# iqbal-lab-org/gramtools

Hardware: AMD Instinct MI355X
Metric: 150bp reads quasimapped/sec (whole node); bit-exact coverage (higher is better)
Workload: dtype u32

## Files before the change

gramtools_amd/csrc/gmx_engine_cover_kernels.h:

```cpp
#pragma once
struct CoverAcc {
  uint32_t *acc;
  uint32_t *log;
  uint32_t *log_cursor;
  uint32_t log_cap;
  uint32_t *scratch_big;
  uint32_t n_lanes_big;
  int rng_mode;
  uint32_t log_sites;
  uint32_t *heap;
  uint64_t heap_words;
  const uint32_t *status;
  uint32_t n_tasks;
  unsigned long long *stats;
};

#define GMX_LOG_PAD 0xFFFFFFFFu
#ifdef GMX_LOOP_STATS
__device__ unsigned long long gmx_cover_stats[6 * 16];
__device__ unsigned long long gmx_coop_stats[6 * 8];
extern "C" int gmx_debug_coop_stats(unsigned long long *out, int reset) {
  if (hipMemcpyFromSymbol(out, HIP_SYMBOL(gmx_coop_stats), sizeof(gmx_coop_stats)) != hipSuccess) return -1;
  if (reset) {
    unsigned long long z[6 * 8] = {0};
// ... 798 lines not shown
    gmx_cover_single_rec<NESTED>(ix, o, acc, recs_in[i], o.cover_overflow_list, 4u);
}

__global__ void gmx_stats_limbs_kernel(unsigned long long *stats, uint32_t *limbs, int recombine) {
  const uint32_t t = threadIdx.x;
  if (!recombine) {
    if (t < 20) limbs[t] = (uint32_t)((stats[t >> 2] >> (16 * (t & 3))) & 0xFFFFull);
    else if (t < 32) limbs[t] = 0;
  } else if (t < 5) {
    unsigned long long v = 0;
    for (int l = 3; l >= 0; --l) v = (v << 16) + limbs[4 * t + l];
    stats[t] = v;
  }
}

#define GMX_PACK_READS 128
#define GMX_PACK_IN_BYTES (24 * 1024)
#define GMX_PACK_OUT_PAIRS (GMX_PACK_IN_BYTES / 32 + GMX_PACK_READS + 8)
typedef uint32_t __attribute__((aligned(1))) gmx_u32_unaligned;
__device__ __forceinline__ void pack4(uint32_t x, uint32_t &lo, uint32_t &hi, uint32_t &bad) {
  uint32_t y = x - 0x01010101u;
  bad |= ((y & ~x & 0x80808080u) | (y & 0xFCFCFCFCu));
  lo = (((y & 0x01010101u) * 0x01020408u) >> 24) & 0xFu;
  hi = ((((y >> 1) & 0x01010101u) * 0x01020408u) >> 24) & 0xFu;
}
__device__ __forceinline__ uint2 pack_tail(const uint8_t *p, uint32_t rem, uint32_t &bad) {
  uint2 out = make_uint2(0, 0);
  for (uint32_t j = 0; j < rem; ++j) {
    uint32_t x = p[j];
    if (x < 1 || x > 4) bad = 1;
// ... 94 lines not shown
```

gramtools_amd/csrc/gmx_engine_host.h:

```cpp
#pragma once
#define HIP_TRY(expr)                                                                      \
  do {                                                                                     \
    hipError_t _e = (expr);                                                                \
    if (_e != hipSuccess) {                                                                \
      gmx_set_error(std::string(#expr) + ": " + hipGetErrorString(_e));                    \
      return GMX_EHIP;                                                                     \
    }                                                                                      \
  } while (0)

enum : int { GMX_TK_SEED = 0, GMX_TK_FILTER0, GMX_TK_FILTER1, GMX_TK_SINGLE, GMX_TK_EXTEND2, GMX_TK_UNPACK, GMX_TK_N };
static_assert(GMX_TK_N <= GMX_TIMED_KERNELS, "gmx_timing::kernel_ms holds GMX_TIMED_KERNELS entries");

struct gmx_engine {
  gmx_engine_opts opts;
  GmxIndexView dview;
  std::vector<void *> allocs;
  uint64_t index_bytes = 0;
  uint32_t *d_fused = nullptr, *d_limbs = nullptr;
  size_t n_fused = 0, n_acc = 0;
  std::vector<uint32_t> phys_allele, phys_pb, phys_grouped;
  std::vector<uint32_t> hit_fix;
  unsigned long long *d_stats = nullptr;
  uint32_t *d_error = nullptr;
  uint32_t *d_log = nullptr, *d_log_cursor = nullptr;
  uint32_t log_cap = 0;
  uint32_t n_allele = 0, n_pb = 0, n_grouped = 0;
  uint64_t cap_reads = 0;
  uint8_t *d_skip = nullptr;
  uint2 *d_packed = nullptr;
  uint64_t cap_packed = 0;
  uint32_t *d_status = nullptr, *d_n_final = nullptr, *d_mapped = nullptr, *d_overflow = nullptr, *d_counters = nullptr;
  uint32_t *d_general_rest = nullptr;
  uint32_t *d_single_rest = nullptr;
  bool cover_jump = false;
  uint32_t *d_task_lists = nullptr;
  GmxSeed *d_alive_seed = nullptr;
  uint32_t *d_alive = nullptr, *d_dead = nullptr, *d_dead2 = nullptr;
  uint64_t *d_seed_cursor = nullptr;
// ... 129 lines not shown
    return GMX_OK;
  }
  int upload(const uint32_t **dst, const gmx::WordBuf &src) {
    uint32_t *q = nullptr;
    int rc = alloc(&q, src.size(), false);
    if (rc) return rc;
    const size_t piece = (size_t)1 << 28;
    for (size_t at = 0; at < src.size(); at += piece)
      HIP_TRY(hipMemcpy(q + at, src.data() + at, std::min(piece, src.size() - at) * sizeof(uint32_t), hipMemcpyHostToDevice));
    index_bytes += src.size() * sizeof(uint32_t);
    *dst = q;
    return GMX_OK;
  }
};

static hipError_t gmx_event_wait(hipEvent_t ev) {
  static const bool spin = getenv("GMX_WAIT_SPIN") != nullptr;
  if (spin) return hipEventSynchronize(ev);
  const auto t0 = std::chrono::steady_clock::now();
  for (bool napping = false;;) {
    const hipError_t q = hipEventQuery(ev);
    if (q != hipErrorNotReady) return q;
    (void)hipGetLastError();
    if (!napping) {
      napping = std::chrono::steady_clock::now() - t0 > std::chrono::microseconds(60);
      continue;
    }
    struct timespec ts = {0, 50 * 1000};
    nanosleep(&ts, nullptr);
  }
}

static int gmx_quiesce(gmx_engine *e) {
  if (!e->ev_wait) HIP_TRY(hipEventCreateWithFlags(&e->ev_wait, hipEventDisableTiming | hipEventBlockingSync));
  hipStream_t streams[5] = {e->last_stream, e->copy_stream, e->side_stream, e->side2_stream, e->copy_stream2};
  for (int i = 0; i < 5; ++i) {
    if (i > 0 && !streams[i]) continue;
    bool seen = false;
    for (int j = 0; j < i; ++j) seen = seen || streams[j] == streams[i];
    if (seen) continue;
// ... 9 lines not shown
  HIP_TRY(hipEventRecord(e->ev_zeroed, stream));
  ++e->zero_epoch;
  return GMX_OK;
}
static int twin_join(gmx_engine *e, hipStream_t stream) {
  gmx_engine *tw = e->twin;
  if (!tw || !e->twin_in_flight) return GMX_OK;
  if (!e->ev_twin_done) HIP_TRY(hipEventCreateWithFlags(&e->ev_twin_done, hipEventDisableTiming));
  HIP_TRY(hipEventRecord(e->ev_twin_done, tw->main_stream));
  HIP_TRY(hipStreamWaitEvent(stream, e->ev_twin_done, 0));
  return GMX_OK;
}
static int flush_reset(gmx_engine *e) {
  if (!e->reset_pending) return GMX_OK;
  e->reset_pending = false;
  HIP_TRY(hipMemsetAsync(e->d_fused, 0, (e->n_fused + 32) * 4, e->reset_stream));
  return note_zeroed(e, e->reset_stream);
}

static int log_settle(gmx_engine *e);
static int gmx_log_drain(gmx_engine *e, uint64_t keep_below) {
  int frc = flush_reset(e);
  if (frc) return frc;
  HIP_TRY(hipDeviceSynchronize());
  uint32_t used = 0;
  HIP_TRY(hipMemcpy(&used, e->d_log_cursor, 4, hipMemcpyDeviceToHost));
  used = std::min(used, e->log_cap);
  e->log_reads_since = 0;
  e->log_known = used;
  if (used <= keep_below) return GMX_OK;
  std::vector<uint32_t> w(used);
  HIP_TRY(hipMemcpy(w.data(), e->d_log, (size_t)used * 4, hipMemcpyDeviceToHost));
  std::vector<uint32_t> key;
  for (size_t i = 0; i < w.size();) {
    if (w[i] == GMX_LOG_PAD) {
      ++i;
      continue;
    }
    if (i + 2 > w.size() || i + 2 + (size_t)w[i + 1] > w.size()) {
      gmx_set_error("grouped-allele-count log: malformed record at word " + std::to_string(i) + " of " + std::to_string(w.size()));
      return GMX_EREF;
    }
    key.assign(1, w[i]);
    key.insert(key.end(), w.begin() + i + 2, w.begin() + i + 2 + w[i + 1]);
    e->log_counts[key] += 1;
    i += 2 + w[i + 1];
  }
  HIP_TRY(hipMemset(e->d_log_cursor, 0, 4));
  e->log_known = 0;
  return GMX_OK;
}

template <class Env, int LIST>
static void launch_cover_lds(gmx_engine *e, hipStream_t stream, const BatchView &b, const SearchOut &o, const CoverAcc &acc,
                             bool after_coop = false) {
  static const uint32_t lanes_env = getenv("GMX_COVER_LANES") ? (uint32_t)atoi(getenv("GMX_COVER_LANES")) : 0u;
  const uint32_t lanes = lanes_env ? std::min(lanes_env, gmx_cover_lds_lanes<Env>()) : gmx_cover_lds_lanes<Env>();
  const size_t lds = (size_t)GmxScratchFixed<Env>::total * lanes * sizeof(uint32_t);
  const uint32_t per_cu = std::min<uint32_t>((uint32_t)(160 * 1024 / lds), 32u);
  hipLaunchKernelGGL((gmx_cover_kernel<Env, LIST>), dim3(e->n_cus * per_cu), dim3(64), lds, stream, e->dview, b, o, e->big,
                     acc, lanes, after_coop ? 1u : 0u);
}

// ... 69 lines not shown
  if ((rc = e->alloc(&e->d_inst_width, e->big.max_slots, false))) return rc;
  if ((rc = e->alloc(&e->d_inst_serial, e->big.max_slots, false))) return rc;
  if ((rc = e->alloc(&e->d_general_serial, n_tasks, false))) return rc;
  if ((rc = e->alloc(&e->d_big_serial, e->big.max_slots, false))) return rc;
  if ((rc = e->alloc(&e->d_overflow3, 2 * n_tasks, false))) return rc;
  if ((rc = e->alloc(&e->d_inst_arena, (size_t)e->inst_cap * GMX_FAST_ARENA, false))) return rc;
  if ((rc = e->alloc(&e->d_inst_states, (size_t)e->inst_cap * GMX_INST_STATES, false))) return rc;
  e->cap_reads = cap;
  return GMX_OK;
}

struct GmxDeviceIndex {
  uint64_t serial = 0;
  int device = 0;
  GmxIndexView view{};
  std::vector<void *> allocs;
  uint64_t bytes = 0;
  int refs = 0;
};
static std::mutex g_dev_index_mu;
static std::vector<GmxDeviceIndex *> g_dev_indexes;
static void gmx_dev_index_release(GmxDeviceIndex *d) {
  if (!d) return;
  std::lock_guard<std::mutex> lk(g_dev_index_mu);
  if (--d->refs > 0) return;
  for (void *p : d->allocs) (void)hipFree(p);
  g_dev_indexes.erase(std::remove(g_dev_indexes.begin(), g_dev_indexes.end(), d), g_dev_indexes.end());
  delete d;
}

static int engine_create(const gmx_index *ixh, const gmx_engine_opts *opts_in, gmx_engine *primary, gmx_engine **out);
int gmx_engine_create(const gmx_index *ixh, const gmx_engine_opts *opts_in, gmx_engine **out) try {
  int rc = engine_create(ixh, opts_in, nullptr, out);
  if (rc) return rc;
  gmx_engine *e = *out;
  const gmx::HostIndex &h = gmx_index_host(ixh);
  const bool can = !e->log_sites && e->shared_index && !getenv("GMX_NO_INDEX_SHARE");
  bool want = can && (h.is_nested || e->index_bytes >= (2ull << 30));
  if (const char *tw = getenv("GMX_TWIN")) want = can && atoi(tw) != 0;
  if (want) {
    gmx_engine *t = nullptr;
    if (engine_create(ixh, &e->opts, e, &t) == GMX_OK) {
      e->twin = t;
// ... 96 lines not shown
  }
  e->dview = v;
  e->n_allele = h.n_allele_slots;
  e->n_pb = h.n_pb_slots;
  e->n_grouped = h.n_grouped_slots;
  {
    e->n_acc = ((size_t)h.n_acc_slots + 63) / 64 * 64;
    e->n_fused = e->n_acc + 32;
    if (primary)
      e->d_fused = primary->d_fused;
    else
      rc |= e->alloc(&e->d_fused, e->n_fused + 32, true);
    e->d_limbs = e->d_fused ? e->d_fused + e->n_acc : nullptr;
    e->d_stats = e->d_fused ? reinterpret_cast<unsigned long long *>(e->d_fused + e->n_fused) : nullptr;
    e->d_log_cursor = e->d_fused ? e->d_fused + e->n_fused + 16 : nullptr;
    rc |= e->alloc(&e->d_error, 2, true);
    e->phys_allele = h.phys_allele;
    e->phys_pb = h.phys_pb;
    e->phys_grouped = h.phys_grouped;
    e->hit_fix = h.hit_fix;
  }
  for (const GmxSite &st : h.sites) e->log_sites = e->log_sites || st.grouped_off == GMX_GROUPED_LOG;
  {
    uint64_t n_jump = 0;
    for (const GmxSiteGeo &g : h.site_geo) n_jump += (g.flags & GMX_SITE_JUMP) ? 1u : 0u;
    e->cover_jump = !h.is_nested && 2 * n_jump > h.site_geo.size() && !getenv("GMX_NO_COVER_JUMP");
    if (getenv("GMX_NO_COVER_JUMP")) e->dview.site_geo = nullptr;
  }
  {
    uint64_t cap = opts.log_cap_words ? opts.log_cap_words
                   : e->log_sites     ? (1ull << 26)
                                      : 64;
    e->log_cap = (uint32_t)std::min<uint64_t>(cap, 0xFFFFFF00ull);
  }
  if (primary)
// ... 84 lines not shown
  }
  if (!primary && e->seed_cursor && !rc && !getenv("GMX_NO_SA_CTX")) {
    uint32_t *sc = nullptr;
    if (e->alloc(&sc, h.sa.size(), false) == GMX_OK) {
      hipLaunchKernelGGL(gmx_sa_ctx_kernel, dim3(8192), dim3(256), 0, nullptr, e->dview.sa, e->dview.text, (uint64_t)h.sa.size(), sc);
      if (hipDeviceSynchronize() == hipSuccess) {
        e->dview.sa_ctx = sc;
        e->index_bytes += h.sa.size() * sizeof(uint32_t);
      }
    } else {
      (void)hipGetLastError();
    }
  }
  if (!primary && e->seed_cursor && !rc && !getenv("GMX_NO_SEED_SIDE") && h.seed_words.size() > 1) {
    uint32_t *side = nullptr;
    const size_t n_side = h.seed_words.size() / 4 + 2;
    if (e->alloc(&side, n_side, false) == GMX_OK) {
      hipLaunchKernelGGL(gmx_seed_side_kernel, dim3(8192), dim3(256), 0, nullptr, e->dview.seeds, (uint64_t)h.seeds.size(), e->dview.seed_words,
                         e->dview.seed_shift, side);
      if (h.kmer_size2)
        hipLaunchKernelGGL(gmx_seed_side_kernel, dim3(8192), dim3(256), 0, nullptr, e->dview.seeds2, (uint64_t)h.seeds2.size(), e->dview.seed_words,
                           e->dview.seed_shift, side);
      if (hipDeviceSynchronize() == hipSuccess) {
        e->dview.seed_side = side;
        e->index_bytes += n_side * sizeof(uint32_t);
      }
    } else {
      (void)hipGetLastError();
    }
  }
  auto make_stream = [&](hipStream_t *st) -> bool {
// ... 31 lines not shown
  (void)hipSetDevice(e->opts.device);
  (void)hipDeviceSynchronize();
  if (e->twin) gmx_engine_destroy(e->twin);
  e->twin = nullptr;
  if (e->main_stream) (void)hipStreamDestroy(e->main_stream);
  if (e->ev_zeroed) (void)hipEventDestroy(e->ev_zeroed);
  if (e->ev_twin_done) (void)hipEventDestroy(e->ev_twin_done);
  if (e->side_stream) (void)hipStreamDestroy(e->side_stream);
  if (e->side2_stream) (void)hipStreamDestroy(e->side2_stream);
  if (e->ev_fork2) (void)hipEventDestroy(e->ev_fork2);
  if (e->ev_side1) (void)hipEventDestroy(e->ev_side1);
  if (e->ev_filter) (void)hipEventDestroy(e->ev_filter);
  if (e->ev_fork) (void)hipEventDestroy(e->ev_fork);
  if (e->ev_join) (void)hipEventDestroy(e->ev_join);
  if (e->ev_wait) (void)hipEventDestroy(e->ev_wait);
  if (e->copy_stream) (void)hipStreamDestroy(e->copy_stream);
  if (e->copy_stream2) (void)hipStreamDestroy(e->copy_stream2);
  if (e->h_log_state) (void)hipHostFree(e->h_log_state);
  if (e->ev_log_state) (void)hipEventDestroy(e->ev_log_state);
  for (auto &sl : e->pslot) {
    if (sl.copied) (void)hipEventDestroy(sl.copied);
    if (sl.done) (void)hipEventDestroy(sl.done);
  }
  for (auto &sl : e->stage) {
    if (sl.copied) (void)hipEventDestroy(sl.copied);
    if (sl.done) (void)hipEventDestroy(sl.done);
    if (sl.h_offsets) (void)hipHostFree(sl.h_offsets);
    if (sl.h_seeds) (void)hipHostFree(sl.h_seeds);
  }
  for (void *p : e->allocs) (void)hipFree(p);
  gmx_dev_index_release(e->shared_index);
  delete e;
} GMX_GUARD_VOID("gmx_engine_destroy")

int gmx_engine_reset(gmx_engine *e) try {
  HIP_TRY(hipSetDevice(e->opts.device));
  e->reset_pending = false;
  HIP_TRY(hipDeviceSynchronize());
  HIP_TRY(hipMemset(e->d_fused, 0, (e->n_fused + 32) * 4));
  HIP_TRY(hipMemset(e->d_error, 0, 8));
  HIP_TRY(hipMemset(e->d_counters, 0, GMX_N_COUNTERS * GMX_CNT_STRIDE * 4));
  if (e->twin) {
    HIP_TRY(hipMemset(e->twin->d_error, 0, 8));
    HIP_TRY(hipMemset(e->twin->d_counters, 0, GMX_N_COUNTERS * GMX_CNT_STRIDE * 4));
    e->twin_in_flight = false;
  }
  e->log_counts.clear();
  e->log_known = e->log_reads_since = 0;
  e->log_state_pending = false;
  return GMX_OK;
} GMX_GUARD_INT("gmx_engine_reset")

int gmx_engine_reset_async(gmx_engine *e, void *hip_stream) try {
  HIP_TRY(hipSetDevice(e->opts.device));
  hipStream_t st = (hipStream_t)hip_stream;
  int frc = flush_reset(e);
  if (frc) return frc;
  if ((frc = twin_join(e, st))) return frc;
  e->twin_in_flight = false;
  e->reset_pending = true;
  e->reset_stream = st;
  e->log_counts.clear();
  e->log_known = e->log_reads_since = 0;
  e->log_state_pending = false;
  return GMX_OK;
} GMX_GUARD_INT("gmx_engine_reset_async")

static bool gmx_ab_no_filter() {
  static const bool off = getenv("GMX_AB_NO_FILTER") != nullptr;
  return off;
}
static void launch_filter(gmx_engine *e, hipStream_t st, dim3 task_grid, const BatchView &b, const SearchOut &o, int pass,
                          hipEvent_t t0 = nullptr, hipEvent_t t1 = nullptr) {
  if (gmx_ab_no_filter()) return;
  if (e->filter_lds_words)
    hipExtLaunchKernelGGL(gmx_filter_lds_kernel, dim3(e->n_cus), dim3(GMX_FILTER_LDS_THREADS), e->filter_lds_words * 4,
// ... 8 lines not shown
  if (!e->h_log_state) {
    HIP_TRY(hipHostMalloc(reinterpret_cast<void **>(&e->h_log_state), 4 * sizeof(uint32_t), hipHostMallocDefault));
    HIP_TRY(hipEventCreateWithFlags(&e->ev_log_state, hipEventDisableTiming));
  }
  HIP_TRY(hipMemcpyAsync(e->h_log_state + 0, e->d_log_cursor, 4, hipMemcpyDeviceToHost, stream));
  HIP_TRY(hipMemcpyAsync(e->h_log_state + 1, e->d_counters + GMX_CNT_LOG_RETRY * GMX_CNT_STRIDE, 4, hipMemcpyDeviceToHost, stream));
  HIP_TRY(hipMemcpyAsync(e->h_log_state + 2, e->d_counters + GMX_CNT_LOG_RETRY_RECS * GMX_CNT_STRIDE, 4, hipMemcpyDeviceToHost, stream));
  HIP_TRY(hipMemcpyAsync(e->h_log_state + 3, e->d_counters + GMX_CNT_LOG_RETRY_HUGE * GMX_CNT_STRIDE, 4, hipMemcpyDeviceToHost, stream));
  HIP_TRY(hipEventRecord(e->ev_log_state, stream));
  e->log_state_pending = true;
  return GMX_OK;
}

static int launch_log_replay(gmx_engine *e, hipStream_t stream) {
  const int in = e->log_retry_side, out = in ^ 1;
  SearchOut o = e->last_o;
  o.log_retry_list = e->d_log_retry[out];
  o.log_retry_recs = e->d_log_retry_recs[out];
  o.log_retry_huge = e->d_log_retry_huge[out];
  o.cover_overflow_list = e->d_log_retry[in];
  hipLaunchKernelGGL(gmx_log_replay_setup_kernel, dim3(1), dim3(1024), 0, stream, o, e->d_log_retry_huge[in]);
  if (e->dview.is_nested)
    hipLaunchKernelGGL(gmx_cover_single_replay_kernel<true>, dim3(e->n_cus * 4), dim3(GMX_BLOCK), 0, stream, e->dview, e->last_b, o, e->last_acc,
                     e->d_log_retry_recs[in]);
  else
    hipLaunchKernelGGL(gmx_cover_single_replay_kernel<false>, dim3(e->n_cus * 4), dim3(GMX_BLOCK), 0, stream, e->dview, e->last_b, o, e->last_acc,
                     e->d_log_retry_recs[in]);
  hipLaunchKernelGGL((gmx_cover_kernel<CoverEnvBig, 1>), dim3(e->cover_big_lanes / 64), dim3(64), e->last_big_lds, stream, e->dview,
                     e->last_b, o, e->big, e->last_acc, 64u, 0u);
  HIP_TRY(hipGetLastError());
// ... 9 lines not shown
  uint64_t before = ~0ull;
  for (int round = 0;; ++round) {
    HIP_TRY(hipEventSynchronize(e->ev_log_state));
    e->log_state_pending = false;
    const uint32_t used = std::min(e->h_log_state[0], e->log_cap);
    const uint64_t retries = (uint64_t)e->h_log_state[1] + e->h_log_state[2] + e->h_log_state[3];
    if (retries == 0) {
      if (used > e->log_cap / 2) return gmx_log_drain(e, 0);
      e->log_known = used;
      return GMX_OK;
    }
    if (round > 0 && retries >= before) {
      HIP_TRY(hipDeviceSynchronize());
      const uint32_t err[2] = {GMX_TASK_LOGFULL, 0};
      HIP_TRY(hipMemcpy(e->d_error, err, 8, hipMemcpyHostToDevice));
      return GMX_OK;
    }
    before = retries;
    int rc = gmx_log_drain(e, 0);
    if (rc) return rc;
    e->log_replays++;
    e->log_replayed_entries += retries;
    if ((rc = launch_log_replay(e, e->last_stream))) return rc;
  }
}

struct BatchInput {
  const uint8_t *d_reads = nullptr;
  const uint64_t *d_offsets = nullptr;
  const uint32_t *d_seeds = nullptr;
// ... 44 lines not shown
    for (uint32_t p = pair; p < n_pairs; ++p) {
      const uint64_t j = base0 + first_base + 32ull * p;
      const uint64_t w = j >> 4;
      const uint32_t sh = (uint32_t)(j & 15u) * 2u;
      const uint32_t w0 = stream[w], w1 = stream[w + 1], w2 = stream[w + 2];
      const unsigned long long bits = (unsigned long long)__builtin_amdgcn_alignbit(w1, w0, sh) |
                                      ((unsigned long long)__builtin_amdgcn_alignbit(w2, w1, sh) << 32);
      out[p] = make_uint2(gmx_even_bits(bits), gmx_even_bits(bits >> 1));
    }
  }
}

static int launch_batch(gmx_engine *e, const BatchInput &in, hipStream_t stream) {
  const uint64_t n_reads = in.n_reads, total_bases = in.total_bases;
  if (n_reads == 0) return GMX_OK;
  if (n_reads > (0x7fffffffull / GMX_FAST_ARENA) / 2) {
    gmx_set_error("batch too large: at most 44 M reads per launch (lower gmx_engine_opts.max_batch_reads)");
    return GMX_EINVAL;
  }
  int rc = e->log_sites ? log_settle(e) : GMX_OK;
  if (rc) return rc;
  if ((rc = ensure_batch_capacity(e, n_reads))) return rc;
  const bool fold_reset = e->reset_pending && e->reset_stream == stream;
  if (e->reset_pending && !fold_reset && (rc = flush_reset(e))) return rc;
  e->reset_pending = false;
  if (!in.d_planes) {
    uint64_t need = total_bases / 32 + n_reads + 16;
    if (need > e->cap_packed) {
      rc = e->alloc(&e->d_packed, need, false);
      if (rc) return rc;
// ... 405 lines not shown
  tw->timing = e->timing;
  out->eng = tw;
  out->stream = tw->main_stream;
  e->twin_in_flight = true;
  e->last_on_twin = true;
  return GMX_OK;
}

static int map_reads_packed_impl(gmx_engine *e, const uint64_t *planes, bool twobit, const uint64_t *offsets, uint32_t uniform_len,
                                 const uint32_t *seeds, const uint8_t *skip, uint64_t n_reads) {
  if (!e || !planes || !seeds || (!offsets && !uniform_len)) {
    gmx_set_error("gmx_map_reads_packed_host / gmx_map_reads_2bit_host: null argument (offsets may be null only with uniform_len)");
    return GMX_EINVAL;
  }
  if (n_reads == 0) return GMX_OK;
  HIP_TRY(hipSetDevice(e->opts.device));
  if (!e->copy_stream) HIP_TRY(hipStreamCreateWithFlags(&e->copy_stream, hipStreamNonBlocking));
  static const bool two_copy_streams = getenv("GMX_TWO_COPY_STREAMS") != nullptr;
  if (two_copy_streams && !e->copy_stream2) HIP_TRY(hipStreamCreateWithFlags(&e->copy_stream2, hipStreamNonBlocking));
  const uint32_t ppr = (uniform_len + 31u) / 32u;
  auto base_at = [&](uint64_t r) -> uint64_t { return uniform_len ? r * uniform_len : offsets[r] - offsets[0]; };
  auto pair_at = [&](uint64_t r) -> uint64_t {
    if (twobit) return (base_at(r) + 31) >> 5;
    return uniform_len ? r * ppr : ((offsets[r] >> 5) - (offsets[0] >> 5)) + r;
  };
  struct Reg { const void *p; bool on; };
  Reg regs[4] = {{planes, false}, {offsets, false}, {seeds, false}, {skip, false}};
  const uint64_t reg_bytes[4] = {pair_at(n_reads) * 8, (n_reads + 1) * 8, n_reads * 4, n_reads};
  bool all_pinned = true;
  for (int i = 0; i < 4; ++i) {
// ... 110 lines not shown
} GMX_GUARD_INT("gmx_map_reads_packed_host")

static uint64_t gmx_feed_chunk(const gmx_engine *e) {
  static const char *env = getenv("GMX_FEED_CHUNK");
  if (env) return std::max<uint64_t>(1, std::min<uint64_t>(e->opts.max_batch_reads, strtoull(env, nullptr, 10)));
  return e->opts.max_batch_reads;
}

int gmx_map_reads_packed_device(gmx_engine *e, const uint64_t *d_planes, const uint64_t *d_offsets, uint32_t uniform_len,
                                const uint32_t *seeds, const uint8_t *d_skip, uint64_t n_reads) try {
  if (!e || !d_planes || !seeds || (!d_offsets && !uniform_len)) {
    gmx_set_error("gmx_map_reads_packed_device: null argument (d_offsets may be null only with uniform_len)");
    return GMX_EINVAL;
  }
  if (n_reads == 0) return GMX_OK;
  HIP_TRY(hipSetDevice(e->opts.device));
  const uint32_t *d_seeds = seeds;
  if (gmx_is_pinned(seeds)) {
    void *dp = nullptr;
    if (hipHostGetDevicePointer(&dp, const_cast<uint32_t *>(seeds), 0) != hipSuccess || !dp) {
      (void)hipGetLastError();
      gmx_set_error("gmx_map_reads_packed_device: the page-locked seeds have no device address");
      return GMX_EHIP;
    }
    d_seeds = static_cast<const uint32_t *>(dp);
  }
  const uint64_t chunk = gmx_feed_chunk(e);
  if (!uniform_len && n_reads > chunk) {
    gmx_set_error("gmx_map_reads_packed_device: with d_offsets a call takes at most 2^20 reads (and at most max_batch_reads)");
    return GMX_EINVAL;
// ... 170 lines not shown
          (rc = e->alloc(&sl.d_skip, n_reads, false)))
        return rc;
      sl.cap_reads = n_reads;
    }
  }
  return GMX_OK;
} GMX_GUARD_INT("gmx_engine_reserve_packed")

int gmx_engine_sync(gmx_engine *e) try {
  HIP_TRY(hipSetDevice(e->opts.device));
  {
    int frc = flush_reset(e);
    if (frc) return frc;
    if ((frc = log_settle(e))) return frc;
  }
  {
    int qrc = gmx_quiesce(e);
    if (qrc) return qrc;
    if (e->twin && (qrc = gmx_quiesce(e->twin))) return qrc;
    e->twin_in_flight = false;
  }
  HIP_TRY(hipStreamSynchronize(e->last_stream));
  HIP_TRY(hipDeviceSynchronize());
  uint32_t c[4] = {0, 0, 0, 0};
  HIP_TRY(hipMemcpy(c + 2, e->d_error, 8, hipMemcpyDeviceToHost));
  if (c[2] == 0 && e->twin) {
    HIP_TRY(hipMemcpy(c + 2, e->twin->d_error, 8, hipMemcpyDeviceToHost));
    if (c[2] != 0) HIP_TRY(hipMemset(e->twin->d_error, 0, 8));
  }
  if (c[2] != 0) {
    HIP_TRY(hipMemset(e->d_error, 0, 8));
    char msg[256];
    if (c[2] == GMX_TASK_LOGFULL) {
      snprintf(msg, sizeof(msg),
               "a read's records exceed the whole grouped-allele-count log (sites without dense group counters; %u words): "
               "nothing of it was recorded: raise gmx_engine_opts.log_cap_words",
               e->log_cap);
      gmx_set_error(msg);
      return GMX_ECAP;
    }
    if (c[2] == GMX_TASK_OVERFLOW) {
      snprintf(msg, sizeof(msg),
               "read %u (orientation %u) needs more memory for its search states or its mapping instances than the whole "
               "last-tier heap holds (%llu bytes); nothing of this read was recorded: raise gmx_engine_opts.huge_heap_bytes "
               "(GMX_HUGE_HEAP_BYTES)",
               c[3] >> 1, c[3] & 1, (unsigned long long)e->heap_words * 4);
// ... 90 lines not shown
  out->log_replays = e->log_replays;
  out->log_replayed_entries = e->log_replayed_entries;
  return GMX_OK;
} GMX_GUARD_INT("gmx_engine_queue_counts")

int gmx_coverage_device(gmx_engine *e, gmx_device_coverage *out) try {
  {
    int frc = flush_reset(e);
    if (frc) return frc;
  }
  if (e->twin && e->twin_in_flight) {
    int qrc = gmx_quiesce(e->twin);
    if (qrc) return qrc;
    e->twin_in_flight = false;
  }
  out->allele_sum = out->per_base = out->grouped = nullptr;
  out->n_allele_sum = e->n_allele;
  out->n_per_base = e->n_pb;
  out->n_grouped = e->n_grouped;
  out->stats = e->d_stats;
  out->n_stats = 5;
  out->fused = e->d_fused;
  out->n_fused = e->n_fused;
  return GMX_OK;
} GMX_GUARD_INT("gmx_coverage_device")

int gmx_coverage_reduce_begin(gmx_engine *e, void *hip_stream) try {
  if (!e) {
    gmx_set_error("null engine");
    return GMX_EINVAL;
  }
  {
    int frc = flush_reset(e);
    if (frc) return frc;
    if ((frc = log_settle(e))) return frc;
  }
  HIP_TRY(hipSetDevice(e->opts.device));
  {
    int trc = twin_join(e, (hipStream_t)hip_stream);
    if (trc) return trc;
  }
  hipLaunchKernelGGL(gmx_stats_limbs_kernel, dim3(1), dim3(64), 0, (hipStream_t)hip_stream, e->d_stats, e->d_limbs, 0);
  HIP_TRY(hipGetLastError());
  return GMX_OK;
} GMX_GUARD_INT("gmx_coverage_reduce_begin")

int gmx_coverage_reduce_end(gmx_engine *e, void *hip_stream) try {
  if (!e) {
    gmx_set_error("null engine");
    return GMX_EINVAL;
  }
  {
    int frc = flush_reset(e);
    if (frc) return frc;
  }
  HIP_TRY(hipSetDevice(e->opts.device));
  hipLaunchKernelGGL(gmx_stats_limbs_kernel, dim3(1), dim3(64), 0, (hipStream_t)hip_stream, e->d_stats, e->d_limbs, 1);
  HIP_TRY(hipGetLastError());
  return GMX_OK;
} GMX_GUARD_INT("gmx_coverage_reduce_end")

int gmx_coverage_fetch(gmx_engine *e, uint32_t *allele_sum, uint32_t *per_base, uint32_t *grouped, gmx_stats *stats) try {
  if (!e) {
    gmx_set_error("null engine");
    return GMX_EINVAL;
  }
  {
    int frc = flush_reset(e);
    if (frc) return frc;
    if ((frc = log_settle(e))) return frc;
  }
  HIP_TRY(hipSetDevice(e->opts.device));
  HIP_TRY(hipDeviceSynchronize());
  std::vector<uint32_t> block(std::max<size_t>(e->n_acc, 1));
  if (e->n_acc) HIP_TRY(hipMemcpy(block.data(), e->d_fused, e->n_acc * 4, hipMemcpyDeviceToHost));
  if (allele_sum) for (size_t i = 0; i < e->phys_allele.size(); ++i) allele_sum[i] = block[e->phys_allele[i]];
  if (per_base) for (size_t i = 0; i < e->phys_pb.size(); ++i) per_base[i] = block[e->phys_pb[i]];
  if (grouped) for (size_t i = 0; i < e->phys_grouped.size(); ++i) grouped[i] = block[e->phys_grouped[i]];
  for (size_t i = 0; i + 3 < e->hit_fix.size(); i += 4) {
    const uint32_t hits = block[e->hit_fix[i]];
    if (allele_sum) allele_sum[e->hit_fix[i + 1]] += hits;
    if (grouped) grouped[e->hit_fix[i + 2]] += hits;
    if (per_base) per_base[e->hit_fix[i + 3]] += hits;
  }
  if (stats) {
    unsigned long long s[5];
    HIP_TRY(hipMemcpy(s, e->d_stats, sizeof(s), hipMemcpyDeviceToHost));
    stats->all_reads_count = s[0];
    stats->skipped_reads_count = s[1];
    stats->missing_kmer_reads_count = s[2];
    stats->no_extension_reads_count = s[3];
    stats->exact_mapped_reads_count = s[4];
  }
  return GMX_OK;
} GMX_GUARD_INT("gmx_coverage_fetch")

int64_t gmx_coverage_fetch_grouped_log(gmx_engine *e, uint32_t *out, uint64_t cap_words) try {
  if (!e) return GMX_EINVAL;
  if (hipSetDevice(e->opts.device) != hipSuccess) return GMX_EHIP;
  if (log_settle(e)) return GMX_EHIP;
  if (gmx_log_drain(e, 0)) return GMX_EHIP;
  uint64_t n = 0;
  for (auto const &kv : e->log_counts) {
    const uint64_t words = 4 + (kv.first.size() - 1);
    if (out && n + words <= cap_words) {
      out[n] = kv.first[0];
      out[n + 1] = (uint32_t)(kv.first.size() - 1) | GMX_LOG_COUNTED;
      out[n + 2] = (uint32_t)kv.second;
      out[n + 3] = (uint32_t)(kv.second >> 32);
      for (size_t j = 1; j < kv.first.size(); ++j) out[n + 3 + j] = kv.first[j];
    }
    n += words;
  }
  return (int64_t)n;
} GMX_GUARD_INT("gmx_coverage_fetch_grouped_log")

// ... 2 lines not shown
    gmx_set_error("gmx_coverage_import_grouped_log: null argument");
    return GMX_EINVAL;
  }
  {
    int frc = flush_reset(e);
    if (frc) return frc;
  }
  HIP_TRY(hipSetDevice(e->opts.device));
  return gmx_engine_log_import(e, records, (size_t)n_words, replace != 0);
} GMX_GUARD_INT("gmx_coverage_import_grouped_log")

}

void gmx_engine_raw(gmx_engine *e, GmxEngineRaw *out) {
  (void)flush_reset(e);
  out->device = e->opts.device;
  out->d_fused = e->d_fused;
  out->n_fused = e->n_fused;
  out->log_sites = e->log_sites;
}

int gmx_engine_log_export(gmx_engine *e, std::vector<uint32_t> &out) {
  {
    int frc = flush_reset(e);
    if (frc) return frc;
    if ((frc = log_settle(e))) return frc;
  }
  const int64_t n = gmx_coverage_fetch_grouped_log(e, nullptr, 0);
  if (n < 0) return (int)n;
  out.assign((size_t)n, 0);
// ... 38 lines not shown
```

gramtools_amd/csrc/gmx_index.h:

```cpp
#pragma once
#include <sys/mman.h>

#include <algorithm>
#include <chrono>
#include <cstdint>
#include <cstdlib>
#include <new>
#include <string>
#include <utility>
#include <vector>

#include "gmx_types.h"

namespace gmx {

inline bool gmx_huge_pages_pay() {
  static const bool ok = [] {
    if (const char *e = getenv("GMX_HUGEPAGES")) return atoi(e) != 0;
    const size_t bytes = (size_t)16 << 20, huge = (size_t)2 << 20;
    auto touch = [&](bool advise) -> double {
      void *p = aligned_alloc(huge, bytes);
      if (!p) return 1e9;
      if (advise && madvise(p, bytes, MADV_HUGEPAGE) != 0) {
        free(p);
// ... 128 lines not shown
  std::vector<uint32_t> l_allele_off, l_grouped_off;
  std::vector<uint32_t> l_cov_off;
  std::vector<uint32_t> phys_allele, phys_pb, phys_grouped;
  std::vector<uint32_t> hit_fix;
  std::vector<uint32_t> site_ref_pos;

  std::vector<uint32_t> bwt;
  std::vector<std::pair<uint32_t, std::vector<TargetedMarker>>> target_map;
  std::vector<std::pair<uint32_t, int32_t>> pos_target;
  uint64_t n_seed_kmers_present = 0;
  uint64_t n_seed_states = 0, n_seed_states_large = 0;

  GmxIndexView view() const;
};

void build_suffix_array(const std::vector<uint32_t> &text, std::vector<uint32_t> &sa, int threads = 1);
void debug_suffix_array_u16(const uint16_t *text, size_t n, uint16_t *sa);

void build_index(const std::vector<uint32_t> &prg, uint32_t kmer_size, HostIndex &out, int threads = 0, int seed_k2 = -1);
void build_index(std::vector<uint32_t> &&prg, uint32_t kmer_size, HostIndex &out, int threads = 0, int seed_k2 = -1);

void save_index(const HostIndex &h, const std::string &path);
void load_index(const std::string &path, const std::vector<uint32_t> &prg, uint32_t kmer_size, HostIndex &out);

std::vector<uint32_t> read_prg_file(const std::string &path);

struct WalkState {
  uint32_t lo, hi, tvd, tvg;
};
struct WalkNode {
// ... 24 lines not shown
```

Baseline: 1.457 billion.

## Gather coverage on device and skip redundant syncs via dirty tracking

Adds a device finalize kernel that gathers the allele, per-base and grouped coverage through precomputed source and hit-fix index tables. It also appends stats, error words and the log cursor as a tail, so the fetch becomes a single staged pinned copy instead of copying the whole accumulator and gathering on the host. Dirty and foreign flags let the error check and log drain skip device-wide synchronisation and extra small memcpys when nothing changed since the last fetch. The twin's error words now sit next to the primary's so both are read in one copy. This adds state-tracking complexity and a risk of stale cached results if any path that modifies device state fails to set the dirty flag.

```diff
diff --git a/gramtools_amd/csrc/gmx_engine_cover_kernels.h b/gramtools_amd/csrc/gmx_engine_cover_kernels.h
--- a/gramtools_amd/csrc/gmx_engine_cover_kernels.h
+++ b/gramtools_amd/csrc/gmx_engine_cover_kernels.h
@@ -836,6 +836,28 @@
   }
 }
 
+#define GMX_FETCH_NO_HIT 0xFFFFFFFFu
+enum : uint32_t { GMX_FETCH_TAIL_STATS = 0, GMX_FETCH_TAIL_ERROR = 10, GMX_FETCH_TAIL_CURSOR = 14, GMX_FETCH_TAIL_WORDS = 16 };
+__global__ void __launch_bounds__(256) gmx_coverage_finalize_kernel(const uint32_t *__restrict__ block, const uint32_t *__restrict__ src,
+                                                                    const uint32_t *__restrict__ hit, uint64_t first, uint32_t n,
+                                                                    uint32_t *__restrict__ out, const uint32_t *stats_words,
+                                                                    const uint32_t *error_words, const uint32_t *log_cursor, uint32_t tail) {
+  for (uint32_t i = blockIdx.x * blockDim.x + threadIdx.x; i < n; i += gridDim.x * blockDim.x) {
+    const uint32_t h = hit[first + i];
+    uint32_t v = block[src[first + i]];
+    if (h != GMX_FETCH_NO_HIT) v += block[h];
+    out[i] = v;
+  }
+  if (tail && blockIdx.x == 0 && threadIdx.x < GMX_FETCH_TAIL_WORDS) {
+    const uint32_t t = threadIdx.x;
+    uint32_t v = 0;
+    if (t < GMX_FETCH_TAIL_ERROR) v = stats_words[t];
+    else if (t < GMX_FETCH_TAIL_CURSOR) v = error_words[t - GMX_FETCH_TAIL_ERROR];
+    else if (t == GMX_FETCH_TAIL_CURSOR) v = *log_cursor;
+    out[n + t] = v;
+  }
+}
+
 #define GMX_PACK_READS 128
 #define GMX_PACK_IN_BYTES (24 * 1024)
 #define GMX_PACK_OUT_PAIRS (GMX_PACK_IN_BYTES / 32 + GMX_PACK_READS + 8)
diff --git a/gramtools_amd/csrc/gmx_engine_host.h b/gramtools_amd/csrc/gmx_engine_host.h
--- a/gramtools_amd/csrc/gmx_engine_host.h
+++ b/gramtools_amd/csrc/gmx_engine_host.h
@@ -22,6 +22,15 @@
   std::vector<uint32_t> hit_fix;
   unsigned long long *d_stats = nullptr;
   uint32_t *d_error = nullptr;
+  const uint32_t *d_fetch_src = nullptr, *d_fetch_hit = nullptr;
+  uint64_t n_fetch = 0;
+  uint32_t *d_fetch_out = nullptr, *h_fetch = nullptr;
+  uint64_t fetch_cap = 0;
+  bool fetch_no_memory = false;
+  hipEvent_t ev_fetch = nullptr;
+  bool dirty = true, foreign = false, errors_clear = false;
+  bool cursor_known = false;
+  uint32_t log_cursor_seen = 0;
   uint32_t *d_log = nullptr, *d_log_cursor = nullptr;
   uint32_t log_cap = 0;
   uint32_t n_allele = 0, n_pb = 0, n_grouped = 0;
@@ -181,7 +190,7 @@
   }
 };
 
-static hipError_t gmx_event_wait(hipEvent_t ev) {
+static hipError_t gmx_event_wait(hipEvent_t ev, int query_us = 60) {
   static const bool spin = getenv("GMX_WAIT_SPIN") != nullptr;
   if (spin) return hipEventSynchronize(ev);
   const auto t0 = std::chrono::steady_clock::now();
@@ -190,7 +199,7 @@
     if (q != hipErrorNotReady) return q;
     (void)hipGetLastError();
     if (!napping) {
-      napping = std::chrono::steady_clock::now() - t0 > std::chrono::microseconds(60);
+      napping = std::chrono::steady_clock::now() - t0 > std::chrono::microseconds(query_us);
       continue;
     }
     struct timespec ts = {0, 50 * 1000};
@@ -230,6 +239,7 @@
 static int flush_reset(gmx_engine *e) {
   if (!e->reset_pending) return GMX_OK;
   e->reset_pending = false;
+  e->dirty = true;
   HIP_TRY(hipMemsetAsync(e->d_fused, 0, (e->n_fused + 32) * 4, e->reset_stream));
   return note_zeroed(e, e->reset_stream);
 }
@@ -238,9 +248,15 @@
 static int gmx_log_drain(gmx_engine *e, uint64_t keep_below) {
   int frc = flush_reset(e);
   if (frc) return frc;
-  HIP_TRY(hipDeviceSynchronize());
   uint32_t used = 0;
-  HIP_TRY(hipMemcpy(&used, e->d_log_cursor, 4, hipMemcpyDeviceToHost));
+  if (!e->dirty && !e->foreign && e->cursor_known) {
+    used = e->log_cursor_seen;
+    if (std::min(used, e->log_cap) <= keep_below) return GMX_OK;
+  } else {
+    HIP_TRY(hipDeviceSynchronize());
+    HIP_TRY(hipMemcpy(&used, e->d_log_cursor, 4, hipMemcpyDeviceToHost));
+  }
+  e->cursor_known = false;
   used = std::min(used, e->log_cap);
   e->log_reads_since = 0;
   e->log_known = used;
@@ -263,6 +279,7 @@
     i += 2 + w[i + 1];
   }
   HIP_TRY(hipMemset(e->d_log_cursor, 0, 4));
+  e->dirty = true;
   e->log_known = 0;
   return GMX_OK;
 }
@@ -362,6 +379,8 @@
   uint64_t serial = 0;
   int device = 0;
   GmxIndexView view{};
+  bool fetch_tried = false;
+  const uint32_t *fetch_src = nullptr, *fetch_hit = nullptr;
   std::vector<void *> allocs;
   uint64_t bytes = 0;
   int refs = 0;
@@ -375,6 +394,43 @@
   for (void *p : d->allocs) (void)hipFree(p);
   g_dev_indexes.erase(std::remove(g_dev_indexes.begin(), g_dev_indexes.end(), d), g_dev_indexes.end());
   delete d;
+}
+
+static bool gmx_fetch_host_gather() {
+  static const bool on = getenv("GMX_FETCH_HOST_GATHER") != nullptr && atoi(getenv("GMX_FETCH_HOST_GATHER")) != 0;
+  return on;
+}
+static void gmx_fetch_tables(gmx_engine *e, const gmx::HostIndex &h) {
+  e->n_fetch = (uint64_t)h.phys_allele.size() + h.phys_pb.size() + h.phys_grouped.size();
+  if (gmx_fetch_host_gather() || e->n_fetch == 0) return;
+  std::lock_guard<std::mutex> share_lock(g_dev_index_mu);
+  GmxDeviceIndex *d = e->shared_index;
+  if (d && d->fetch_tried) {
+    e->d_fetch_src = d->fetch_src;
+    e->d_fetch_hit = d->fetch_hit;
+    return;
+  }
+  if (d) d->fetch_tried = true;
+  std::vector<uint32_t> src, hit;
+  if (!gmx::fetch_tables(h.phys_allele, h.phys_pb, h.phys_grouped, h.hit_fix, h.n_acc_slots, src, hit)) return;
+  std::vector<void *> &owner = d ? d->allocs : e->allocs;
+  owner.reserve(owner.size() + 1);
+  uint32_t *q = nullptr;
+  const size_t n = src.size();
+  if (hipMalloc(reinterpret_cast<void **>(&q), 2 * n * sizeof(uint32_t)) != hipSuccess ||
+      hipMemcpy(q, src.data(), n * sizeof(uint32_t), hipMemcpyHostToDevice) != hipSuccess ||
+      hipMemcpy(q + n, hit.data(), n * sizeof(uint32_t), hipMemcpyHostToDevice) != hipSuccess) {
+    (void)hipGetLastError();
+    if (q) (void)hipFree(q);
+    return;
+  }
+  owner.push_back(q);
+  e->d_fetch_src = q;
+  e->d_fetch_hit = q + n;
+  if (d) {
+    d->fetch_src = e->d_fetch_src;
+    d->fetch_hit = e->d_fetch_hit;
+  }
 }
 
 static int engine_create(const gmx_index *ixh, const gmx_engine_opts *opts_in, gmx_engine *primary, gmx_engine **out);
@@ -501,11 +557,15 @@
     e->d_limbs = e->d_fused ? e->d_fused + e->n_acc : nullptr;
     e->d_stats = e->d_fused ? reinterpret_cast<unsigned long long *>(e->d_fused + e->n_fused) : nullptr;
     e->d_log_cursor = e->d_fused ? e->d_fused + e->n_fused + 16 : nullptr;
-    rc |= e->alloc(&e->d_error, 2, true);
+    if (primary)
+      e->d_error = primary->d_error + 2;
+    else
+      rc |= e->alloc(&e->d_error, 4, true);
     e->phys_allele = h.phys_allele;
     e->phys_pb = h.phys_pb;
     e->phys_grouped = h.phys_grouped;
     e->hit_fix = h.hit_fix;
+    if (!primary && !rc) gmx_fetch_tables(e, h);
   }
   for (const GmxSite &st : h.sites) e->log_sites = e->log_sites || st.grouped_off == GMX_GROUPED_LOG;
   {
@@ -620,7 +680,7 @@
   }
   if (!primary && e->seed_cursor && !rc && !getenv("GMX_NO_SEED_SIDE") && h.seed_words.size() > 1) {
     uint32_t *side = nullptr;
-    const size_t n_side = h.seed_words.size() / 4 + 2;
+    const size_t n_side = h.seed_words.size() / 4 + 2 + 4;
     if (e->alloc(&side, n_side, false) == GMX_OK) {
       hipLaunchKernelGGL(gmx_seed_side_kernel, dim3(8192), dim3(256), 0, nullptr, e->dview.seeds, (uint64_t)h.seeds.size(), e->dview.seed_words,
                          e->dview.seed_shift, side);
@@ -682,6 +742,9 @@
   if (e->ev_fork) (void)hipEventDestroy(e->ev_fork);
   if (e->ev_join) (void)hipEventDestroy(e->ev_join);
   if (e->ev_wait) (void)hipEventDestroy(e->ev_wait);
+  if (e->ev_fetch) (void)hipEventDestroy(e->ev_fetch);
+  if (e->d_fetch_out) (void)hipFree(e->d_fetch_out);
+  if (e->h_fetch) (void)hipHostFree(e->h_fetch);
   if (e->copy_stream) (void)hipStreamDestroy(e->copy_stream);
   if (e->copy_stream2) (void)hipStreamDestroy(e->copy_stream2);
   if (e->h_log_state) (void)hipHostFree(e->h_log_state);
@@ -705,11 +768,13 @@
   HIP_TRY(hipSetDevice(e->opts.device));
   e->reset_pending = false;
   HIP_TRY(hipDeviceSynchronize());
+  e->dirty = true;
+  e->cursor_known = false;
+  e->last_stream = nullptr;
   HIP_TRY(hipMemset(e->d_fused, 0, (e->n_fused + 32) * 4));
-  HIP_TRY(hipMemset(e->d_error, 0, 8));
+  HIP_TRY(hipMemset(e->d_error, 0, 16));
   HIP_TRY(hipMemset(e->d_counters, 0, GMX_N_COUNTERS * GMX_CNT_STRIDE * 4));
   if (e->twin) {
-    HIP_TRY(hipMemset(e->twin->d_error, 0, 8));
     HIP_TRY(hipMemset(e->twin->d_counters, 0, GMX_N_COUNTERS * GMX_CNT_STRIDE * 4));
     e->twin_in_flight = false;
   }
@@ -728,6 +793,8 @@
   e->twin_in_flight = false;
   e->reset_pending = true;
   e->reset_stream = st;
+  e->dirty = true;
+  e->cursor_known = false;
   e->log_counts.clear();
   e->log_known = e->log_reads_since = 0;
   e->log_state_pending = false;
@@ -766,6 +833,7 @@
 
 static int launch_log_replay(gmx_engine *e, hipStream_t stream) {
   const int in = e->log_retry_side, out = in ^ 1;
+  e->dirty = true;
   SearchOut o = e->last_o;
   o.log_retry_list = e->d_log_retry[out];
   o.log_retry_recs = e->d_log_retry_recs[out];
@@ -805,6 +873,8 @@
       HIP_TRY(hipDeviceSynchronize());
       const uint32_t err[2] = {GMX_TASK_LOGFULL, 0};
       HIP_TRY(hipMemcpy(e->d_error, err, 8, hipMemcpyHostToDevice));
+      e->dirty = true;
+      e->errors_clear = false;
       return GMX_OK;
     }
     before = retries;
@@ -879,6 +949,7 @@
 static int launch_batch(gmx_engine *e, const BatchInput &in, hipStream_t stream) {
   const uint64_t n_reads = in.n_reads, total_bases = in.total_bases;
   if (n_reads == 0) return GMX_OK;
+  e->dirty = true;
   if (n_reads > (0x7fffffffull / GMX_FAST_ARENA) / 2) {
     gmx_set_error("batch too large: at most 44 M reads per launch (lower gmx_engine_opts.max_batch_reads)");
     return GMX_EINVAL;
@@ -1314,6 +1385,7 @@
     return GMX_EINVAL;
   }
   if (n_reads == 0) return GMX_OK;
+  e->dirty = true;
   HIP_TRY(hipSetDevice(e->opts.device));
   if (!e->copy_stream) HIP_TRY(hipStreamCreateWithFlags(&e->copy_stream, hipStreamNonBlocking));
   static const bool two_copy_streams = getenv("GMX_TWO_COPY_STREAMS") != nullptr;
@@ -1454,6 +1526,7 @@
     return GMX_EINVAL;
   }
   if (n_reads == 0) return GMX_OK;
+  e->dirty = true;
   HIP_TRY(hipSetDevice(e->opts.device));
   const uint32_t *d_seeds = seeds;
   if (gmx_is_pinned(seeds)) {
@@ -1654,6 +1727,7 @@
     if (frc) return frc;
     if ((frc = log_settle(e))) return frc;
   }
+  if (!e->dirty && !e->foreign && e->errors_clear) return GMX_OK;
   {
     int qrc = gmx_quiesce(e);
     if (qrc) return qrc;
@@ -1662,14 +1736,20 @@
   }
   HIP_TRY(hipStreamSynchronize(e->last_stream));
   HIP_TRY(hipDeviceSynchronize());
-  uint32_t c[4] = {0, 0, 0, 0};
-  HIP_TRY(hipMemcpy(c + 2, e->d_error, 8, hipMemcpyDeviceToHost));
-  if (c[2] == 0 && e->twin) {
-    HIP_TRY(hipMemcpy(c + 2, e->twin->d_error, 8, hipMemcpyDeviceToHost));
-    if (c[2] != 0) HIP_TRY(hipMemset(e->twin->d_error, 0, 8));
-  }
+  uint32_t c[4] = {0, 0, 0, 0}, both[4] = {0, 0, 0, 0};
+  HIP_TRY(hipMemcpy(both, e->d_error, 16, hipMemcpyDeviceToHost));
+  e->dirty = e->foreign = false;
+  c[2] = both[0];
+  c[3] = both[1];
+  if (c[2] == 0 && e->twin && both[2] != 0) {
+    c[2] = both[2];
+    c[3] = both[3];
+    both[2] = 0;
+    HIP_TRY(hipMemset(e->twin->d_error, 0, 8));
+  }
+  e->errors_clear = !(e->twin && both[2] != 0);
   if (c[2] != 0) {
-    HIP_TRY(hipMemset(e->d_error, 0, 8));
+    if (both[0] != 0) HIP_TRY(hipMemset(e->d_error, 0, 8));
     char msg[256];
     if (c[2] == GMX_TASK_LOGFULL) {
       snprintf(msg, sizeof(msg),
@@ -1790,6 +1870,7 @@
     if (qrc) return qrc;
     e->twin_in_flight = false;
   }
+  e->dirty = e->foreign = true;
   out->allele_sum = out->per_base = out->grouped = nullptr;
   out->n_allele_sum = e->n_allele;
   out->n_per_base = e->n_pb;
@@ -1816,6 +1897,7 @@
     int trc = twin_join(e, (hipStream_t)hip_stream);
     if (trc) return trc;
   }
+  e->dirty = e->foreign = true;
   hipLaunchKernelGGL(gmx_stats_limbs_kernel, dim3(1), dim3(64), 0, (hipStream_t)hip_stream, e->d_stats, e->d_limbs, 0);
   HIP_TRY(hipGetLastError());
   return GMX_OK;
@@ -1831,22 +1913,109 @@
     if (frc) return frc;
   }
   HIP_TRY(hipSetDevice(e->opts.device));
+  e->dirty = e->foreign = true;
   hipLaunchKernelGGL(gmx_stats_limbs_kernel, dim3(1), dim3(64), 0, (hipStream_t)hip_stream, e->d_stats, e->d_limbs, 1);
   HIP_TRY(hipGetLastError());
   return GMX_OK;
 } GMX_GUARD_INT("gmx_coverage_reduce_end")
+
+static uint64_t gmx_fetch_stage_words() {
+  static const uint64_t mb = getenv("GMX_FETCH_STAGE_MB") ? std::max<uint64_t>(1, strtoull(getenv("GMX_FETCH_STAGE_MB"), nullptr, 10)) : 64;
+  return std::min<uint64_t>(mb, 2048) << 18;
+}
+
+static int coverage_fetch_device(gmx_engine *e, hipStream_t st, uint32_t *allele_sum, uint32_t *per_base, uint32_t *grouped, gmx_stats *stats,
+                                 bool *done) {
+  *done = false;
+  if (!e->d_fetch_src || e->fetch_no_memory) return GMX_OK;
+  const uint64_t piece_max = gmx_fetch_stage_words() - GMX_FETCH_TAIL_WORDS;
+  const uint64_t need = std::min<uint64_t>(e->n_fetch, piece_max) + GMX_FETCH_TAIL_WORDS;
+  if (need > e->fetch_cap) {
+    if (e->d_fetch_out) (void)hipFree(e->d_fetch_out);
+    if (e->h_fetch) (void)hipHostFree(e->h_fetch);
+    e->d_fetch_out = e->h_fetch = nullptr;
+    e->fetch_cap = 0;
+    if (hipMalloc(reinterpret_cast<void **>(&e->d_fetch_out), need * 4) != hipSuccess ||
+        hipHostMalloc(reinterpret_cast<void **>(&e->h_fetch), need * 4, hipHostMallocDefault) != hipSuccess) {
+      (void)hipGetLastError();
+      if (e->d_fetch_out) (void)hipFree(e->d_fetch_out);
+      e->d_fetch_out = e->h_fetch = nullptr;
+      e->fetch_no_memory = true;
+      return GMX_OK;
+    }
+    e->fetch_cap = need;
+  }
+  if (!e->ev_fetch) HIP_TRY(hipEventCreateWithFlags(&e->ev_fetch, hipEventDisableTiming));
+  const uint32_t *error_words = e->d_error;
+  uint32_t *const dst[3] = {allele_sum, per_base, grouped};
+  const uint64_t len[3] = {e->n_allele, e->n_pb, e->n_grouped};
+  uint32_t n_last = 0;
+  for (uint64_t at = 0;;) {
+    const uint32_t n = (uint32_t)std::min<uint64_t>(e->n_fetch - at, piece_max);
+    const bool last = at + n == e->n_fetch;
+    const uint32_t grid = (uint32_t)std::min<uint64_t>(std::max<uint64_t>((n + 255u) / 256u, 1), (uint64_t)e->n_cus * 8);
+    hipLaunchKernelGGL(gmx_coverage_finalize_kernel, dim3(grid), dim3(256), 0, st, e->d_fused, e->d_fetch_src, e->d_fetch_hit, at, n,
+                       e->d_fetch_out, reinterpret_cast<const uint32_t *>(e->d_stats), error_words, e->d_log_cursor, last ? 1u : 0u);
+    HIP_TRY(hipGetLastError());
+    HIP_TRY(hipMemcpyAsync(e->h_fetch, e->d_fetch_out, ((size_t)n + (last ? GMX_FETCH_TAIL_WORDS : 0u)) * 4, hipMemcpyDeviceToHost, st));
+    HIP_TRY(hipEventRecord(e->ev_fetch, st));
+    HIP_TRY(gmx_event_wait(e->ev_fetch, 1000));
+    uint64_t first = 0;
+    for (int k = 0; k < 3; ++k) {
+      const uint64_t lo = std::max(first, at), hi = std::min(first + len[k], at + n);
+      if (dst[k] && lo < hi) memcpy(dst[k] + (lo - first), e->h_fetch + (lo - at), (hi - lo) * 4);
+      first += len[k];
+    }
+    at += n;
+    n_last = n;
+    if (last) break;
+  }
+  const uint32_t *tail = e->h_fetch + n_last;
+  if (stats) {
+    unsigned long long s[5];
+    memcpy(s, tail + GMX_FETCH_TAIL_STATS, sizeof(s));
+    stats->all_reads_count = s[0];
+    stats->skipped_reads_count = s[1];
+    stats->missing_kmer_reads_count = s[2];
+    stats->no_extension_reads_count = s[3];
+    stats->exact_mapped_reads_count = s[4];
+  }
+  e->errors_clear = tail[GMX_FETCH_TAIL_ERROR] == 0 && tail[GMX_FETCH_TAIL_ERROR + 2] == 0;
+  e->log_cursor_seen = tail[GMX_FETCH_TAIL_CURSOR];
+  e->cursor_known = true;
+  e->twin_in_flight = false;
+  e->dirty = e->foreign = false;
+  *done = true;
+  return GMX_OK;
+}
 
 int gmx_coverage_fetch(gmx_engine *e, uint32_t *allele_sum, uint32_t *per_base, uint32_t *grouped, gmx_stats *stats) try {
   if (!e) {
     gmx_set_error("null engine");
     return GMX_EINVAL;
   }
+  HIP_TRY(hipSetDevice(e->opts.device));
+  const bool reset_elsewhere = e->reset_pending && e->reset_stream != e->last_stream;
   {
     int frc = flush_reset(e);
     if (frc) return frc;
     if ((frc = log_settle(e))) return frc;
   }
-  HIP_TRY(hipSetDevice(e->opts.device));
+  if (!gmx_fetch_host_gather()) {
+    const hipStream_t st = e->last_stream;
+    if (e->foreign) {
+      HIP_TRY(hipDeviceSynchronize());
+    } else if (reset_elsewhere) {
+      if (!e->ev_fetch) HIP_TRY(hipEventCreateWithFlags(&e->ev_fetch, hipEventDisableTiming));
+      HIP_TRY(hipEventRecord(e->ev_fetch, e->reset_stream));
+      HIP_TRY(hipStreamWaitEvent(st, e->ev_fetch, 0));
+    }
+    int trc = twin_join(e, st);
+    if (trc) return trc;
+    bool done = false;
+    if ((trc = coverage_fetch_device(e, st, allele_sum, per_base, grouped, stats, &done))) return trc;
+    if (done) return GMX_OK;
+  }
   HIP_TRY(hipDeviceSynchronize());
   std::vector<uint32_t> block(std::max<size_t>(e->n_acc, 1));
   if (e->n_acc) HIP_TRY(hipMemcpy(block.data(), e->d_fused, e->n_acc * 4, hipMemcpyDeviceToHost));
@@ -1875,7 +2044,7 @@
   if (!e) return GMX_EINVAL;
   if (hipSetDevice(e->opts.device) != hipSuccess) return GMX_EHIP;
   if (log_settle(e)) return GMX_EHIP;
-  if (gmx_log_drain(e, 0)) return GMX_EHIP;
+  if (e->log_sites && gmx_log_drain(e, 0)) return GMX_EHIP;
   uint64_t n = 0;
   for (auto const &kv : e->log_counts) {
     const uint64_t words = 4 + (kv.first.size() - 1);
@@ -1908,6 +2077,7 @@
 
 void gmx_engine_raw(gmx_engine *e, GmxEngineRaw *out) {
   (void)flush_reset(e);
+  e->dirty = e->foreign = true;
   out->device = e->opts.device;
   out->d_fused = e->d_fused;
   out->n_fused = e->n_fused;
diff --git a/gramtools_amd/csrc/gmx_index.h b/gramtools_amd/csrc/gmx_index.h
--- a/gramtools_amd/csrc/gmx_index.h
+++ b/gramtools_amd/csrc/gmx_index.h
@@ -166,6 +166,30 @@
   GmxIndexView view() const;
 };
 
+inline bool fetch_tables(const std::vector<uint32_t> &phys_allele, const std::vector<uint32_t> &phys_pb, const std::vector<uint32_t> &phys_grouped,
+                         const std::vector<uint32_t> &hit_fix, uint32_t n_acc_slots, std::vector<uint32_t> &src, std::vector<uint32_t> &hit) {
+  const size_t na = phys_allele.size(), np = phys_pb.size(), ng = phys_grouped.size();
+  src.clear();
+  src.reserve(na + np + ng);
+  src.insert(src.end(), phys_allele.begin(), phys_allele.end());
+  src.insert(src.end(), phys_pb.begin(), phys_pb.end());
+  src.insert(src.end(), phys_grouped.begin(), phys_grouped.end());
+  for (uint32_t s : src)
+    if (s >= n_acc_slots) return false;
+  hit.assign(src.size(), 0xFFFFFFFFu);
+  if (hit_fix.size() % 4 != 0) return false;
+  for (size_t i = 0; i < hit_fix.size(); i += 4) {
+    const uint32_t counter = hit_fix[i], a = hit_fix[i + 1], g = hit_fix[i + 2], p = hit_fix[i + 3];
+    if (counter >= n_acc_slots || a >= na || g >= ng || p >= np) return false;
+    uint32_t *slots[3] = {&hit[a], &hit[na + p], &hit[na + np + g]};
+    for (uint32_t *slot : slots) {
+      if (*slot != 0xFFFFFFFFu) return false;
+      *slot = counter;
+    }
+  }
+  return true;
+}
+
 void build_suffix_array(const std::vector<uint32_t> &text, std::vector<uint32_t> &sa, int threads = 1);
 void debug_suffix_array_u16(const uint16_t *text, size_t n, uint16_t *sa);
 
```

New measurement: 1.455 billion. No clear change (-0.2%).
